# baycom/tfrec

Hardware: AMD Instinct MI355X
Metric: IQ MSamples/s through demod+decode (batched streams) (higher is better)
Workload: dtype int32+f32+f64

## Files before the change

### include/tfrec_amd.h

```cpp
#ifndef TFREC_AMD_H
#define TFREC_AMD_H

#include <stddef.h>
#include <stdint.h>

#ifdef __cplusplus
extern "C" {
#endif

#define TFREC_AMD_BLOCK_BYTES 65536
#define TFREC_AMD_FIFO_DEPTH 4
#define TFREC_AMD_BLOCK_BYTES_10X 655360
#define TFREC_AMD_BLOCK_DEC 8192
#define TFREC_AMD_NSLOTS 5

enum { TFREC_AMD_SLOT_TFA1 = 0, TFREC_AMD_SLOT_TFA2 = 1, TFREC_AMD_SLOT_TFA3 = 2, TFREC_AMD_SLOT_TX22 = 3,
       TFREC_AMD_SLOT_WHB = 4 };

enum {
	TFREC_AMD_OK = 0,
	TFREC_AMD_E_INVAL = -1,
	TFREC_AMD_E_NOMEM = -2,
	TFREC_AMD_E_HIP = -3,
	TFREC_AMD_E_OVERFLOW = -4,
// ... 271 lines not shown
int tfrec_amd_rssi_db(int slot, int64_t rssi_raw);

int tfrec_amd_read_stage0(tfrec_amd_ctx *ctx, int stream, int16_t *out, size_t n_pairs);
int tfrec_amd_read_decimated(tfrec_amd_ctx *ctx, int stream, int16_t *out, size_t n_pairs);
typedef struct {
	uint64_t resolved;
	uint64_t host_verified;
	uint64_t host_mismatch;
	uint64_t undecidable;
	uint64_t reserved[4];
} tfrec_amd_fm_stats;
int tfrec_amd_get_fm_stats(tfrec_amd_ctx *ctx, tfrec_amd_fm_stats *out);
int tfrec_amd_atan_uncertain(tfrec_amd_ctx *ctx, uint64_t *n);
int tfrec_amd_fm_dev_probe(int device, int kind, const void *records, size_t n, int32_t *out, tfrec_amd_fm_stats *stats);
int tfrec_amd_iir_probe(int device, double cutoff, int form, const double *in, size_t n, double *out);
int tfrec_amd_read_biquad_row(tfrec_amd_ctx *ctx, int slot, int stream, int32_t *out, size_t cap_values, uint32_t *n_slots);
int tfrec_amd_get_timings(tfrec_amd_ctx *ctx, tfrec_amd_timings *out);
typedef struct {
	uint64_t biquad_segments;
	uint64_t biquad_unconverged;
	uint64_t biquad_serial;
	uint64_t tfa2_resliced;
	uint64_t tfa1_recomputed;
	uint64_t biquad_repair_slots;
	uint64_t whb_respeculated;
	uint64_t tfa1_scalar_groups;
	uint64_t tfa2_scalar_groups;
	uint64_t tfa1_vector_groups;
	uint64_t tfa2_vector_groups;
} tfrec_amd_stats;
// ... 10 lines not shown
```

### tfrec_amd/api.py

```python
from __future__ import annotations

import ctypes as C
import os
from fractions import Fraction

import numpy as np

from . import _build
from .burst import BURST_DTYPE
from .capture import RUN_DTYPE
from .clock import CLOCK_DTYPE
from .envelope import ENVELOPE_DTYPE
from .levels import LEVEL_DTYPE
from .occupancy import OCC_DTYPE
from .sync import SYNC_DTYPE
from .track import TRACK_DTYPE

BLOCK_BYTES = 65536
BLOCK_DEC = 8192
NSLOTS = 5
FIFO_DEPTH = 4
SLOT_NAMES = ("TFA_1", "TFA_2", "TFA_3", "TX22", "WHB")

F_ALL_FLUSHES = 1
# ... 72 lines not shown
    "tfrec_amd_get_timings", "tfrec_amd_read_thresh", "tfrec_amd_get_stats", "tfrec_amd_get_layout", "tfrec_amd_host_alloc",
    "tfrec_amd_host_free", "tfrec_amd_read_stage0", "tfrec_amd_get_fm_stats", "tfrec_amd_fm_dev_probe",
    "tfrec_amd_fifo_depth", "tfrec_amd_get_memory", "tfrec_amd_iir_probe", "tfrec_amd_reset_streams",
    "tfrec_amd_configure_streams", "tfrec_amd_get_stream_config", "tfrec_amd_tune_streams", "tfrec_amd_get_stream_tune",
    "tfrec_amd_map_streams", "tfrec_amd_get_stream_input", "tfrec_amd_tune_streams_wide", "tfrec_amd_get_stream_tune_wide",
    "tfrec_amd_create_rate", "tfrec_amd_get_input_rate", "tfrec_amd_input_bytes", "tfrec_amd_resample_taps",
    "tfrec_amd_tune_streams_input", "tfrec_amd_get_stream_tune_input", "tfrec_amd_create_format", "tfrec_amd_get_input_format",
    "tfrec_amd_read_levels", "tfrec_amd_enable_capture", "tfrec_amd_read_captures", "tfrec_amd_enable_spectrum",
    "tfrec_amd_read_spectrum", "tfrec_amd_enable_occupancy", "tfrec_amd_read_occupancy", "tfrec_amd_create_dc", "tfrec_amd_get_dc",
    "tfrec_amd_read_dc", "tfrec_amd_reset_dc_rows", "tfrec_amd_create_iq", "tfrec_amd_get_iq", "tfrec_amd_read_iq", "tfrec_amd_reset_iq_rows", "tfrec_amd_create_decimated", "tfrec_amd_enable_capture_pre",
    "tfrec_amd_read_capture_pre", "tfrec_amd_enable_runs_input", "tfrec_amd_submit_runs", "tfrec_amd_read_biquad_row",
    "tfrec_amd_enable_burst_meter", "tfrec_amd_read_bursts", "tfrec_amd_stream_state_bytes", "tfrec_amd_save_streams",
    "tfrec_amd_load_streams", "tfrec_amd_enable_burst_envelope", "tfrec_amd_read_burst_envelopes",
    "tfrec_amd_enable_burst_clock", "tfrec_amd_read_burst_clocks",
    "tfrec_amd_enable_burst_track", "tfrec_amd_set_burst_track_centre", "tfrec_amd_read_burst_tracks",
    "tfrec_amd_enable_burst_sync", "tfrec_amd_read_burst_syncs",
)

_libs = {}


def library_path(experiments: bool = False, short_segments: bool = False) -> str:
    return _build.VARIANTS[_build.variant_name(experiments, short_segments)][0]


def load_library(build: bool = True, experiments: bool = False, short_segments: bool = False):
    key = _build.variant_name(experiments, short_segments)
    if key in _libs:
        return _libs[key]
    if build:
        try:
# ... 23 lines not shown
    L.tfrec_amd_pending_events.argtypes = [C.c_void_p, C.POINTER(C.c_int)]
    L.tfrec_amd_rssi_db.argtypes = [C.c_int, C.c_int64]
    L.tfrec_amd_rssi_db.restype = C.c_int
    L.tfrec_amd_read_decimated.argtypes = [C.c_void_p, C.c_int, C.c_void_p, C.c_size_t]
    L.tfrec_amd_read_stage0.argtypes = [C.c_void_p, C.c_int, C.c_void_p, C.c_size_t]
    L.tfrec_amd_read_biquad_row.argtypes = [C.c_void_p, C.c_int, C.c_int, C.c_void_p, C.c_size_t, C.POINTER(C.c_uint32)]
    L.tfrec_amd_atan_uncertain.argtypes = [C.c_void_p, C.POINTER(C.c_uint64)]
    L.tfrec_amd_get_timings.argtypes = [C.c_void_p, C.POINTER(Timings)]
    L.tfrec_amd_read_thresh.argtypes = [C.c_void_p, C.c_int, C.POINTER(C.c_int)]
    L.tfrec_amd_get_stats.argtypes = [C.c_void_p, C.POINTER(Stats)]
    L.tfrec_amd_get_layout.argtypes = [C.c_void_p, C.POINTER(C.c_int)]
    L.tfrec_amd_get_memory.argtypes = [C.c_void_p, C.POINTER(C.c_uint64), C.POINTER(C.c_uint64)]
    L.tfrec_amd_get_fm_stats.argtypes = [C.c_void_p, C.POINTER(FmStats)]
    L.tfrec_amd_fm_dev_probe.argtypes = [C.c_int, C.c_int, C.c_void_p, C.c_size_t, C.c_void_p, C.POINTER(FmStats)]
    L.tfrec_amd_iir_probe.argtypes = [C.c_int, C.c_double, C.c_int, C.c_void_p, C.c_size_t, C.c_void_p]
    L.tfrec_amd_reset_streams.argtypes = [C.c_void_p, C.c_void_p, C.c_int]
    L.tfrec_amd_configure_streams.argtypes = [C.c_void_p, C.c_void_p, C.c_void_p, C.c_int]
    L.tfrec_amd_get_stream_config.argtypes = [C.c_void_p, C.c_int, C.POINTER(StreamConfig)]
    L.tfrec_amd_tune_streams.argtypes = [C.c_void_p, C.c_void_p, C.c_void_p, C.c_int]
    L.tfrec_amd_get_stream_tune.argtypes = [C.c_void_p, C.c_int, C.POINTER(C.c_int32)]
    L.tfrec_amd_map_streams.argtypes = [C.c_void_p, C.c_void_p, C.c_void_p, C.c_int]
    L.tfrec_amd_get_stream_input.argtypes = [C.c_void_p, C.c_int, C.POINTER(C.c_int32)]
    L.tfrec_amd_tune_streams_wide.argtypes = [C.c_void_p, C.c_void_p, C.c_void_p, C.c_int]
    L.tfrec_amd_get_stream_tune_wide.argtypes = [C.c_void_p, C.c_int, C.POINTER(C.c_int32)]
    L.tfrec_amd_tune_streams_input.argtypes = [C.c_void_p, C.c_void_p, C.c_void_p, C.c_int]
    L.tfrec_amd_get_stream_tune_input.argtypes = [C.c_void_p, C.c_int, C.POINTER(C.c_int32)]
    L.tfrec_amd_create_rate.argtypes = [C.POINTER(Config), C.c_int32, C.c_int32, C.POINTER(C.c_void_p)]
    L.tfrec_amd_get_input_rate.argtypes = [C.c_void_p, C.POINTER(C.c_int32), C.POINTER(C.c_int32)]
    L.tfrec_amd_input_bytes.argtypes = [C.c_void_p, C.c_int, C.POINTER(C.c_size_t)]
    L.tfrec_amd_resample_taps.argtypes = [C.c_int32, C.c_int32, C.c_void_p, C.c_int, C.POINTER(C.c_int)]
# ... 591 lines not shown
    L = load_library()
    q = np.ascontiguousarray(records, dtype=np.int32).reshape(-1, 4)
    out = np.empty(len(q), dtype=np.int32)
    _check(L, L.tfrec_amd_fm_dev_probe(device, 2, q.ctypes.data, len(q), out.ctypes.data, None))
    return out


def iir_probe(cutoff: float, x: np.ndarray, form: int = 1, device: int = 0) -> np.ndarray:
    L = load_library()
    xin = np.ascontiguousarray(x, dtype=np.float64)
    out = np.empty(len(xin), dtype=np.float64)
    _check(L, L.tfrec_amd_iir_probe(device, float(cutoff), int(form), xin.ctypes.data, len(xin), out.ctypes.data))
    return out


def fm_dev_probe(records: np.ndarray, device: int = 0, cross: bool = False):
    L = load_library()
    q = (np.ascontiguousarray(records, dtype=np.int64).reshape(-1, 2) if cross
         else np.ascontiguousarray(records, dtype=np.int32).reshape(-1, 4))
    out = np.empty(len(q), dtype=np.int32)
    st = FmStats()
    _check(L, L.tfrec_amd_fm_dev_probe(device, 1 if cross else 0, q.ctypes.data, len(q), out.ctypes.data, C.byref(st)))
    return out, {n: int(getattr(st, n)) for n, _ in FmStats._fields_[:4]}


def events_canon(events: np.ndarray):
    L = load_library()
    events = events[events["status"] != STATUS_BITS]
    m = np.empty((len(events), 71), dtype=np.int64)
    m[:, 0] = events["slot"]
# ... 47 lines not shown
```

### tfrec_amd/csrc/capi_create.h

```cpp
#pragma once

static BiquadCoef biquad_coef(double cutoff)
{
	static const struct {
		double cutoff, b0, a1, a2;
	} known[] = {
		{ 0.5 / (384000.0 / 17240), 0x1.27f98b1037a14p-8, 0x1.cd1527f4a26e2p+0, -0x1.a36a1c41c6995p-1 },
		{ 0.5 / (384000.0 / 9600), 0x1.7ed02b18a270dp-10, 0x1.e397ac010fc89p+0, -0x1.ca2cf85850d62p-1 },
		{ 0.5 / (384000.0 / 8842), 0x1.461fa1a309718p-10, 0x1.e5d4f47377e30p+0, -0x1.ce36282a35d90p-1 },
		{ 2.0 / 64.0, 0x1.14a67102a1ffdp-7, 0x1.b949652fa3970p+0, -0x1.83dd316f714e0p-1 },
		{ 0.0025 / 64.0, 0x1.02ae4cfc8910ap-26, 0x1.ffe9409fe171bp+0, -0x1.ffd283451f7d3p-1 },
	};
	BiquadCoef c;
	for (const auto &k : known)
		if (k.cutoff == cutoff) {
			c.b0 = k.b0;
			c.b1 = k.b0 + k.b0;
			c.b2 = k.b0;
			c.a1 = k.a1;
			c.a2 = k.a2;
			return c;
		}
	const double i = 1.0 / tan(cutoff * M_PI);
	const double s = sqrt(2.0);
// ... 519 lines not shown
	hipStream_t cp = nullptr;
	TRY(own_stream(c, S.fs, prio_hi));
	TRY(own_stream(c, cp, 0));
	TRY(own_stream(c, S.cs, prio_hi));
	S.ws = S.fs;
	c->cpy = cp;
	if (c->cfg.flags & TFREC_AMD_F_SERIAL_CHAINS)
		return TFREC_AMD_OK;
	TRY(own_stream(c, S.t1, prio_hi));
	TRY(own_stream(c, S.aux, prio_hi));
	const char *dp = TFREC_KNOB_STR("DEEP");
	c->deep = dp ? atoi(dp) != 0 : true;
	c->fmdev_k2 = has_kind(c->launch, 1) && has_kind(c->launch, 2);
	S.k2 = S.cs;
	S.kw = S.aux;
	S.vx = S.aux;
	if (!c->deep)
		return TFREC_AMD_OK;
	TRY(own_stream(c, S.k2, 0));
	TRY(own_stream(c, S.kw, 0));
	S.ws = S.kw;
	if (c->fmdev_k2) {
		TRY(own_stream(c, S.fq, prio_lo));
		TRY(own_stream(c, S.ks, prio_lo));
	}
	TRY(own_stream(c, c->cpy, prio_lo));
	S.vx = cp;
	return TFREC_AMD_OK;
}

static int make_pipes(tfrec_amd_ctx *c, const PipeCtl &S)
{
	const bool serial = (c->cfg.flags & TFREC_AMD_F_SERIAL_CHAINS) != 0;
	const bool timing = (c->cfg.flags & TFREC_AMD_F_TIMING) != 0;
	for (int k = 0; k < kSets; k++) {
		PipeCtl &P = c->pipe[k];
		P = S;
		for (hipEvent_t *e : { &P.done[0], &P.done[1], &P.done[2], &P.ev_win, &P.ev_fork, &P.ev_k2, &P.ev_kw, &P.ev_fm,
				       &P.ev_spec, &c->ev_in[k], &P.ev_front, &c->copied[k] })
			TRY(own_event(c, *e, hipEventDisableTiming));
		if (!serial)
			TRY(own_event(c, P.ev_aux, hipEventDisableTiming));
		if (timing) {
			for (hipEvent_t &e : c->ev[k])
				TRY(own_event(c, e, hipEventDefault));
			if (!serial) {
				for (hipEvent_t &e : c->tev[k])
					TRY(own_event(c, e, hipEventDefault));
				P.tev = c->tev[k];
			}
		}
		P.whb_carry = c->d_whbcarry;
		P.fmdev_wmax = c->fmdev_k2 ? c->wmax : 0;
		P.fm_flag_eps = c->fm_flag_eps;
	}
	return TFREC_AMD_OK;
}
// ... 165 lines not shown
```

### tfrec_amd/csrc/capi_probe.h

```cpp
#pragma once

static void account_fm_log(FmTotals *t, const EventBuf &eb)
{
	t->resolved += eb.uncertain;
	t->undecidable += eb.fm_undecidable;
	const uint32_t n = std::min<uint32_t>(eb.fm_logged, (uint32_t)kFmLogCap);
	const double scale = 16384.0 * (1.0 / M_PI);
	for (uint32_t k = 0; k < n; k++) {
		const int want = d2i_host(atan2(eb.fm_log[k].cj, eb.fm_log[k].cr) * scale);
		t->verified++;
		if (want != eb.fm_log[k].result)
			t->mismatch++;
	}
}

static void report_debug_stats(tfrec_amd_ctx *c, int set, int n_blocks)
{
#ifdef TFREC_AMD_VECSTAT
	if (c->submit_seq == 3) {
		(void)hipDeviceSynchronize();
		unsigned long long st[16] = { 0 };
		(void)hipMemcpy(st, c->win[set].stats, sizeof(st), hipMemcpyDeviceToHost);
		fprintf(stderr, "VECSTAT (one submit) TFA_1: groups %llu, stale piece %llu, entered-with-none hazard %llu, > 64 bits in a lane %llu, lanes with 32 ones or more %llu; TFA_2 family: groups %llu, entered with relative 0 %llu, > 16 rounds %llu, > 64 bits in a lane %llu, walks of the groups that converged %llu\n", st[8], st[9], st[10], st[11], st[5], st[12], st[13], st[14], st[15], st[6]);
	}
// ... 207 lines not shown
		return TFREC_AMD_E_INVAL;
	HIPCHK(hipSetDevice(device));
	double *d_in = nullptr, *d_out = nullptr;
	int rc = TFREC_AMD_OK;
	if (hipMalloc((void **)&d_in, n * 8) != hipSuccess || hipMalloc((void **)&d_out, n * 8) != hipSuccess)
		rc = TFREC_AMD_E_NOMEM;
	if (rc == TFREC_AMD_OK && (hipMemcpy(d_in, in, n * 8, hipMemcpyHostToDevice) != hipSuccess ||
				   launch_iir_probe(nullptr, d_in, n, biquad_coef(cutoff), d_out, form) != hipSuccess ||
				   hipMemcpy(out, d_out, n * 8, hipMemcpyDeviceToHost) != hipSuccess))
		rc = hip_fail(hipGetLastError(), "iir_probe");
	(void)hipFree(d_in);
	(void)hipFree(d_out);
	return rc;
}

int tfrec_amd_read_thresh(tfrec_amd_ctx *c, int stream, int *thresh)
{
	if (!c || !thresh || stream < 0 || stream >= c->cfg.n_streams)
		return TFREC_AMD_E_INVAL;
	if (!c->settings.per_stream && c->cfg.thresh) {
		*thresh = c->cfg.thresh;
		return TFREC_AMD_OK;
	}
	TRY(tfrec_amd_sync(c));
	FskState f;
	HIPCHK(hipMemcpy(&f, c->d_fsk + stream, sizeof(f), hipMemcpyDeviceToHost));
	*thresh = f.thresh;
	return TFREC_AMD_OK;
}

// ... 117 lines not shown
```

### tfrec_amd/csrc/chains2.hip

```cpp
#include <stdlib.h>

#include <algorithm>

#include "decoder_dev.h"
#include "launch.h"
#include <type_traits>
#include "whb_chain_asm.h"

namespace tfrec {

constexpr int kSpecLbi = -(1 << 30);

__device__ __forceinline__ int whb_hook_perturb(const WinTables &T)
{
#ifdef TFREC_AMD_EXPERIMENTS
	return T.whb_test_perturb;
#else
	return 0;
#endif
}
__device__ __forceinline__ int whb_hook_force_fail(const WinTables &T)
{
#ifdef TFREC_AMD_EXPERIMENTS
	return T.whb_force_fail;
// ... 166 lines not shown
					whb_spec = a;
				}
				mark(kMarkWhbDemodEnd, P.aux);
				mark(kMarkWhbDecodeEnd, P.aux);
				mark(kMarkWhbCommitEnd, P.aux);
			}
	}
	if (whb_spec >= 0) {
		if (P.vx != P.aux) {
			TRY(hipEventRecord(P.ev_aux, P.aux));
			TRY(hipStreamWaitEvent(P.vx, P.ev_aux, 0));
		}
		mark(kMarkWhbCheck, P.vx);
		hipLaunchKernelGGL(whb_chain_kernel, dim3((n_streams + kChkStreams - 1) / kChkStreams), dim3(64 * (1 + kChkProducers)), kChkLdsBytes,
				   P.vx, n_streams, L, whb_spec, T);
		hipLaunchKernelGGL(whb_check_kernel, dim3(n_streams), block, 0, P.vx, n_streams, L, whb_spec, T, P.whb_carry);
		ChainLaunch Lr = L;
		WinTables Tr = T;
		Tr.whbpub = L.states[whb_spec];
		Lr.states[whb_spec] = T.whbscr;
		hipLaunchKernelGGL((whb_demod_kernel<true, true>), dim3((n_streams + 63) / 64), block, 64 * 64, P.vx, dec, dec_stride, dev32, n_streams,
				   n_blocks, sample_base, Lr, whb_spec, Tr, events, eb, flags);
		mark(kMarkWhbCheckEnd, P.vx);
		TRY(hipEventRecord(P.done[1], P.vx));
	} else {
		TRY(hipEventRecord(P.done[1], P.aux));
	}
	static_assert(kMarkTfa2End == kMarkTfa2Coop + 3 && kMarkTfa1End == kMarkTfa1Coop + 3, "a slicer chain's marks are consecutive");
	auto slicer_chain = [&](int kind, hipStream_t s_, int m0) {
		if (kind == 0)
			hipLaunchKernelGGL(mark_kernel, dim3(std::max(1, win_blocks / 16)), dim3(256), 0, s_, dec, dec_stride, n_streams,
					   n_blocks, L, T);
		const size_t slds = (kind == 0 ? 8 : 4) * 64 * sizeof(uint4);
		hipLaunchKernelGGL(slicer_kernel, dim3(std::max(64, win_blocks)), block, slds, s_, dec, dec_stride, ld16, n_streams, n_blocks, L, T,
				   lanes, head_chunks, kind, 0);
		mark(m0, s_);
		hipLaunchKernelGGL(coop_slicer_kernel, dim3(coop_blocks), block, 0, s_, dec, dec_stride, ld16, n_streams, n_blocks, L,
				   T, kind);
		mark(m0 + 1, s_);
// ... 56 lines not shown
			TRY(hipStreamWaitEvent(P.t1, P.ev_win, 0));
		mark(kMarkTfa1Slicer, P.t1);
		slicer_chain(0, P.t1, kMarkTfa1Coop);
	}
	TRY(hipEventRecord(P.done[2], P.t1));
#undef TRY
	return hipGetLastError();
}

hipError_t whb_chain_lds_optin()
{
	return hipFuncSetAttribute(reinterpret_cast<const void *>(&whb_chain_kernel), hipFuncAttributeMaxDynamicSharedMemorySize,
				   (int)kChkLdsBytes);
}

}
```

### tfrec_amd/csrc/launch.h

```cpp
#pragma once

namespace tfrec {

struct FrontOut {
	uint32_t *dec;             size_t dec_stride;
	unsigned long long *mask;  size_t mask_stride;
	uint32_t *prevdec;
	int16_t *fmdev;            size_t fmdev_stride;
	int n_streams, n_blocks;
};
struct History {
	const uint8_t *in;
	uint8_t *out;
};
struct RateTable {
	int p, q, t;
	const float *taps;
};
struct CaptureBufs {
	CaptureState *state;
	CaptureStage *stage;
	int stage_cap;
	uint2 *cnt;
	uint4 *base;
// ... 53 lines not shown
hipError_t launch_burst_meter(hipStream_t st, const FrontOut &o, const CaptureBufs &b, tfrec_amd_burst *out);
hipError_t launch_burst_envelope(hipStream_t st, const FrontOut &o, const CaptureBufs &b, tfrec_amd_envelope *out);
hipError_t launch_burst_clock(hipStream_t st, const FrontOut &o, const CaptureBufs &b, tfrec_amd_clock *out);
hipError_t launch_burst_track(hipStream_t st, const FrontOut &o, const CaptureBufs &b, const TrackBufs &k);
hipError_t launch_burst_sync(hipStream_t st, const FrontOut &o, const CaptureBufs &b, const SyncBufs &k);
hipError_t launch_spectrum(hipStream_t st, int fmt, const uint8_t *iq, size_t stride, const SpectrumBufs &b);
hipError_t launch_occupancy(hipStream_t st, const SpectrumBufs &b, uint32_t ratio, uint32_t rel, tfrec_amd_occupancy *recs, uint32_t *bits);
hipError_t launch_fm_probe(hipStream_t st, const int32_t *quads, size_t n, int32_t *out, EventBuf *eb, int kind);
hipError_t launch_iir_probe(hipStream_t st, const double *in, size_t n, const BiquadCoef &c, double *out, int form);
hipError_t launch_chains(hipStream_t st, const FrontOut &o, long long sample_base, const ChainLaunch &L, tfrec_amd_event *events,
			 EventBuf *eb, uint32_t flags);
hipError_t launch_threshold(hipStream_t st, const FrontOut &o, FskState *fsk, int wmax, const StreamCfg *scfg);
hipError_t launch_pipeline(const PipeCtl &P, const FrontOut &o, long long sample_base, const ChainLaunch &L, const WinTables &T, int16_t *ld16,
			   int32_t *dev32, tfrec_amd_event *events, EventBuf *eb, uint32_t flags);
hipError_t whb_chain_lds_optin();
struct StateTable;
hipError_t launch_stream_state(hipStream_t st, bool load, const StateTable &T, const int32_t *list, int n_list, uint8_t *stage);

}
```

### tfrec_amd/csrc/tfrec_dev.h

```cpp
#pragma once

#include <hip/hip_runtime.h>
#include <stddef.h>
#include <stdint.h>

#include "../../include/tfrec_amd.h"

#if defined(__HIP_DEVICE_COMPILE__)
#if !defined(__gfx950__)
#error "tfrec_amd: the device code targets gfx950 (MI355X) only"
#endif
#if defined(__AMDGCN_WAVEFRONT_SIZE) && __AMDGCN_WAVEFRONT_SIZE != 64
#error "tfrec_amd: the device code assumes 64-lane wavefronts"
#endif
#endif

namespace tfrec {

constexpr int kBlockDec = TFREC_AMD_BLOCK_DEC;
constexpr int kIndexSpan = 2 * kBlockDec;
constexpr int kTailBytes = 112;
constexpr int kNSlots = TFREC_AMD_NSLOTS;
constexpr int kFmtU8 = TFREC_AMD_FMT_U8, kFmtS8 = TFREC_AMD_FMT_S8, kFmtS16 = TFREC_AMD_FMT_S16, kFmtF32 = TFREC_AMD_FMT_F32;
constexpr int kFmtDec16 = TFREC_AMD_FMT_DEC16;
// ... 299 lines not shown
	ChainState *whbscr;
	ChainState *whbpub;
	int32_t whb_test_perturb;
	int32_t tfa2_vec;
	int32_t tfa1_vec;
};
constexpr int kStatusDead = 0xff;

struct PipeCtl {
	hipStream_t fs;
	hipStream_t ws;
	hipEvent_t ev_front;
	hipStream_t k2, kw;
	hipStream_t cs, aux, t1;
	hipStream_t vx;
	hipEvent_t ev_aux;
	int *whb_carry;
	hipEvent_t ev_win;
	hipEvent_t ev_fork;
	hipEvent_t ev_k2, ev_kw;
	hipEvent_t ev_fm;
	hipStream_t fq;
	hipStream_t ks;
	hipEvent_t ev_spec;
	hipEvent_t done[3];
	hipEvent_t *tev;
	int fmdev_wmax;
	double fm_flag_eps;
};
enum TimingMark : int {
	kMarkWindows = 0,
// ... 35 lines not shown
```

### tfrec_amd/csrc/whb_check.h

```cpp
#pragma once

#ifndef TFREC_AMD_CHK_STREAMS
#define TFREC_AMD_CHK_STREAMS 32
#endif
constexpr int kChkStreams = TFREC_AMD_CHK_STREAMS;
constexpr int kChkProducers = 2;
constexpr int kChkPerProducer = kChkStreams / kChkProducers;
static_assert(kChkStreams <= 64 && kChkStreams % kChkProducers == 0, "a lane per stream, the streams split evenly");
constexpr int kChkPairRow = 64 * 4 + 4;
constexpr int kChkDevRow = 64 + 4;
struct ChkBuf {
	uint32_t pair[kChkStreams * kChkPairRow];
	uint32_t dev[kChkStreams * kChkDevRow];
};
constexpr size_t kChkLdsBytes = 2 * sizeof(ChkBuf);

__global__ __launch_bounds__(64 * (1 + kChkProducers)) void whb_chain_kernel(int n_streams, ChainLaunch L, int a, WinTables T)
{
	extern __shared__ __attribute__((aligned(16))) uint8_t chk_lds[];
	ChkBuf *const buf = reinterpret_cast<ChkBuf *>(chk_lds);
	const int wave = (int)threadIdx.x >> 6, ln = (int)threadIdx.x & 63;
	const int s0 = (int)blockIdx.x * kChkStreams;
	const ChainParams &p = L.params[a];
	const double a1 = p.iir_avg.a1, a2 = p.iir_avg.a2, bh = 0.5 * p.iir_avg.b0;
	const int my_s = s0 + ln;
	const bool my_on = ln < kChkStreams && my_s < n_streams;
	const int my_rounds = my_on ? T.whbdense_n[my_s] >> 6 : 0;
	int rmax = my_rounds;
#pragma unroll
	for (int o = 32; o >= 1; o >>= 1) {
		const int other = __shfl_xor(rmax, o, 64);
		rmax = other > rmax ? other : rmax;
	}
	rmax = __builtin_amdgcn_readfirstlane(rmax);
	if (rmax == 0)
		return;
	if (wave == 0) {
		double y1 = 0.0, y2 = 0.0;
		if (my_on) {
			const WhbExact st = T.whbx[my_s];
			y1 = st.y1;
			y2 = st.y2;
		}
		unsigned long long *const xbits = T.whbxbits + (size_t)(my_on ? my_s : 0) * T.whbx_stride;
		double2 *const xsnap = T.whbxsnap + (size_t)(my_on ? my_s : 0) * T.whbx_stride;
		__syncthreads();
		for (int r = 0; r < rmax; r++) {
			if (r < my_rounds) {
				const ChkBuf &b = buf[r & 1];
				const double2 *prow = reinterpret_cast<const double2 *>(b.pair + ln * kChkPairRow);
				const uint4 *drow = reinterpret_cast<const uint4 *>(b.dev + ln * kChkDevRow);
				uint32_t acc[2] = { 0u, 0u };
				double2 pq[2][8];
				uint4 dq[2][2];
				auto fetch = [&](int h, int g8) {
#pragma unroll
					for (int j = 0; j < 8; j++)
						pq[h][j] = prow[8 * g8 + j];
					dq[h][0] = drow[2 * g8];
					dq[h][1] = drow[2 * g8 + 1];
// ... 8 lines not shown
							    (int)dq[h][1].x, (int)dq[h][1].y, (int)dq[h][1].z, (int)dq[h][1].w };
#pragma unroll
					for (int j = 0; j < 8; j++) {
						const double P = pq[h][j].x, B2 = pq[h][j].y;
						const double y = ((B2 + a1 * y1) + P) + a2 * y2;
						y2 = y1;
						y1 = y;
						const int yi = (int)y;
						asm("v_cmp_lt_i32 vcc, %1, %2\n\tv_addc_co_u32 %0, vcc, %0, %0, vcc" : "+v"(acc[g8 >> 2]) : "v"(dv[j]), "v"(yi) : "vcc");
					}
				}
				xbits[r] = (unsigned long long)__brev(acc[0]) | ((unsigned long long)__brev(acc[1]) << 32);
				xsnap[r] = make_double2(y1, y2);
			}
			__syncthreads();
		}
	} else {
		const int q0 = (wave - 1) * kChkPerProducer;
		int rounds[kChkPerProducer], h1[kChkPerProducer], h2[kChkPerProducer];
		const int32_t *row[kChkPerProducer];
#pragma unroll
		for (int q = 0; q < kChkPerProducer; q++) {
			const int s = s0 + q0 + q;
			const bool on = s < n_streams;
			rounds[q] = __builtin_amdgcn_readlane(my_rounds, (q0 + q) & 63);
			row[q] = T.whbdense + (size_t)(on ? s : 0) * T.whbdense_stride;
			const WhbExact st = T.whbx[on ? s : 0];
			h1[q] = __builtin_amdgcn_readfirstlane(st.fd1);
			h2[q] = __builtin_amdgcn_readfirstlane(st.fd2);
		}
// ... 9 lines not shown
				if (r < rounds[q]) {
					const int d0 = cur[q];
					const int s1 = __builtin_amdgcn_update_dpp(0, d0, 0x138, 0xf, 0xf, false);
					const int d1 = ln == 0 ? h1[q] : s1;
					const int s2 = __builtin_amdgcn_update_dpp(0, d1, 0x138, 0xf, 0xf, false);
					const int d2 = ln == 0 ? h2[q] : s2;
					const double t0 = bh * (double)d0, t1 = bh * (double)d1, t2 = bh * (double)d2;
					const double P = __builtin_fma(2.0, t1, t0);
					*reinterpret_cast<double2 *>(b.pair + (q0 + q) * kChkPairRow + 4 * ln) = make_double2(P, t2);
					b.dev[(q0 + q) * kChkDevRow + ln] = (uint32_t)d0;
					h1[q] = __builtin_amdgcn_readlane(d0, 63);
					h2[q] = __builtin_amdgcn_readlane(d0, 62);
				}
			}
		};
		lay_out(buf[0], 0);
		__syncthreads();
		for (int r = 0; r < rmax; r++) {
			int far[kChkPerProducer];
#pragma unroll
			for (int q = 0; q < kChkPerProducer; q++)
				far[q] = r + 2 < rounds[q] ? row[q][64 * (r + 2) + ln] : 0;
#pragma unroll
			for (int q = 0; q < kChkPerProducer; q++)
				cur[q] = nxt[q];
			if (r + 1 < rmax)
				lay_out(buf[(r + 1) & 1], r + 1);
#pragma unroll
			for (int q = 0; q < kChkPerProducer; q++)
				nxt[q] = far[q];
			__syncthreads();
		}
	}
}

constexpr int kChkLockCap = 256;
__global__ __launch_bounds__(64) void whb_check_kernel(int n_streams, ChainLaunch L, int a, WinTables T, int *__restrict__ carry_io)
{
	__shared__ int lk_pos[kChkLockCap], lk_avgf[kChkLockCap];
	__shared__ uint32_t lk_meta[kChkLockCap];
	const int s = (int)blockIdx.x, ln = (int)threadIdx.x;
	if (s >= n_streams)
		return;
	const ChainParams &p = L.params[a];
	const double a1 = p.iir_avg.a1, a2 = p.iir_avg.a2, bh = 0.5 * p.iir_avg.b0;
	const int N = T.whbdense_n[s], R = N >> 6;
	const int32_t *dense = T.whbdense + (size_t)s * T.whbdense_stride;
	const unsigned long long *xbits = T.whbxbits + (size_t)s * T.whbx_stride;
	const double2 *xsnap = T.whbxsnap + (size_t)s * T.whbx_stride;
	const WhbExact st0 = T.whbx[s];
	const int tp_ = whb_hook_perturb(T);
	const int tol = tp_ > 1 ? tp_ : (tp_ < -1 ? -tp_ : 1);
	auto input = [&](int pos) -> int { return pos >= 0 ? dense[pos] : (pos == -1 ? st0.fd1 : st0.fd2); };
	auto run = [&](int rr, int cnt, double &y1, double &y2, unsigned long long &bits) {
		const int p0 = 64 * rr;
		if (rr == 0) {
			y1 = st0.y1;
			y2 = st0.y2;
		} else {
			const double2 sn = xsnap[rr - 1];
			y1 = sn.x;
			y2 = sn.y;
		}
		double t1 = bh * (double)input(p0 - 1), t2 = bh * (double)input(p0 - 2);
		bits = 0ull;
		for (int k = 0; k < cnt; k++) {
			const int d = dense[p0 + k];
			const double t0 = bh * (double)d;
			const double P = __builtin_fma(2.0, t1, t0);
			const double y = ((t2 + a1 * y1) + P) + a2 * y2;
			bits |= (unsigned long long)(d < (int)y ? 1u : 0u) << k;
			y2 = y1;
			y1 = y;
			t2 = t1;
			t1 = t0;
		}
	};
	double yf1 = 0.0, yf2 = 0.0;
	unsigned long long tailbits = 0ull;
	if (ln == 0)
		run(R, N & 63, yf1, yf2, tailbits);
	tailbits = __shfl(tailbits, 0, 64);
	auto word = [&](int i) -> unsigned long long { return i < R ? xbits[i] : (i == R ? tailbits : 0ull); };
	const uint4 *recrow = reinterpret_cast<const uint4 *>(T.whbrec + (size_t)s * T.whbrec_stride);
	int carry = carry_io[s];
	const int carry_in = carry;
	bool bad = false;
	int cbase = 0, nlocks = 0;
	bool ended = false;
	int last_delta = 0;
	bool have_last = false, last_closed = false;
	auto do_locks = [&]() {
		for (int b0 = 0; b0 < nlocks; b0 += 64) {
			const int i = b0 + ln;
			const bool on = i < nlocks;
			double y1 = 0.0, y2 = 0.0;
			unsigned long long bits;
			const int pos = on ? lk_pos[i] : 0;
			run(pos >> 6, on ? (pos & 63) + 1 : 0, y1, y2, bits);
			const uint32_t meta = on ? lk_meta[i] : 0u;
			const int delta = (int)y1 - (on ? lk_avgf[i] : 0);
			const bool b = on && (delta > tol || delta < -tol || (delta != 0 && (meta & kWhbRecAmb)));
			bad = bad || __ballot(b) != 0ull;
			const int nb = nlocks - b0 < 64 ? nlocks - b0 : 64;
			last_delta = __shfl(delta, nb - 1, 64);
			last_closed = (__shfl((int)meta, nb - 1, 64) & (int)kWhbRecClosed) != 0;
			have_last = true;
		}
		nlocks = 0;
	};
	for (int v0 = 0; !ended; v0 += 64) {
		const int vi = v0 + ln < T.whbrec_stride - 1 ? v0 + ln : T.whbrec_stride - 1;
		const uint4 rec = recrow[vi];
		const uint32_t meta = rec.z;
		const unsigned long long endm = __ballot(meta == kWhbRecEnd);
		const int nrec = endm ? __builtin_ctzll(endm) : 64;
		ended = endm != 0ull || v0 + 64 + 64 > T.whbrec_stride;
		const bool on = ln < nrec;
		const bool pseudo = on && (meta & kWhbRecPseudo) != 0u;
		const bool normal = on && !pseudo;
		const int nv = normal ? (int)((meta >> kWhbRecNvShift) & 63u) + 1 : 0;
		int inc = nv;
#pragma unroll
		for (int o = 1; o < 64; o <<= 1) {
			const int up = __shfl_up(inc, o, 64);
			inc += ln >= o ? up : 0;
		}
		const int pos0 = cbase + inc - nv;
		cbase += __shfl(inc, 63, 64);
		if (pseudo) {
			if (v0 + ln == 0) {
				bad = bad || (carry != 0 && (meta & kWhbRecAmb));
// ... 20 lines not shown
				const int i = nlocks + __builtin_popcountll(lm & ((1ull << ln) - 1ull));
				lk_pos[i] = pos0 + nv - 1;
				lk_avgf[i] = (int)rec.w;
				lk_meta[i] = meta;
			}
			nlocks += __builtin_popcountll(lm);
			__syncthreads();
		}
	}
	if (nlocks)
		do_locks();
	bad = __ballot(bad) != 0ull || cbase != N;
	if (have_last)
		carry = last_closed ? 0 : last_delta;
	if (ln == 0) {
		WhbExact st = st0;
		st.carry = carry_in;
		st.pad_ = 0;
		T.whbx0[s] = st;
		bad = bad || T.whbseen[s] != T.whbgen[s];
		if (whb_hook_force_fail(T) > 0 && (s + T.whb_submit_seq) % whb_hook_force_fail(T) == 0)
			bad = true;
		st.y1 = yf1;
		st.y2 = yf2;
		st.fd1 = input(N - 1);
		st.fd2 = input(N - 2);
		st.carry = st.pad_ = 0;
		T.whbx[s] = st;
		carry_io[s] = bad ? 0 : carry;
		T.whbfail[s] = bad ? 1 : 0;
	}
}
```

Measured before the change: 308,000.

## Move WHB tail recursion into chain kernel and allow check on separate stream

The chain kernel now processes the partial final 64-sample group of each WHB stream, writes its tail bits and end state, and saves the start state in whbx0. This removes the serial lane-0 tail loop and state writeback from the check kernel. An optional knob can place the check and demod kernels on a separate or copy stream behind an event, so they may overlap with other work. A probe entry point is added for testing the chain kernel. The default stream placement is unchanged, so only the moved tail computation affects the default path.

```diff
diff --git a/include/tfrec_amd.h b/include/tfrec_amd.h
--- a/include/tfrec_amd.h
+++ b/include/tfrec_amd.h
@@ -309,6 +309,9 @@
 int tfrec_amd_atan_uncertain(tfrec_amd_ctx *ctx, uint64_t *n);
 int tfrec_amd_fm_dev_probe(int device, int kind, const void *records, size_t n, int32_t *out, tfrec_amd_fm_stats *stats);
 int tfrec_amd_iir_probe(int device, double cutoff, int form, const double *in, size_t n, double *out);
+int tfrec_amd_whb_chain_probe(int device, int n_streams, int stride, double a1, double a2, double b0, const int32_t *seq,
+			      const int32_t *n, const double *y_start, const int32_t *fd_start, uint64_t *bits, double *snap,
+			      double *y_end, int32_t *fd_end, double *y_seen, int32_t *fd_seen);
 int tfrec_amd_read_biquad_row(tfrec_amd_ctx *ctx, int slot, int stream, int32_t *out, size_t cap_values, uint32_t *n_slots);
 int tfrec_amd_get_timings(tfrec_amd_ctx *ctx, tfrec_amd_timings *out);
 typedef struct {
diff --git a/tfrec_amd/api.py b/tfrec_amd/api.py
--- a/tfrec_amd/api.py
+++ b/tfrec_amd/api.py
@@ -110,7 +110,7 @@
     "tfrec_amd_load_streams", "tfrec_amd_enable_burst_envelope", "tfrec_amd_read_burst_envelopes",
     "tfrec_amd_enable_burst_clock", "tfrec_amd_read_burst_clocks",
     "tfrec_amd_enable_burst_track", "tfrec_amd_set_burst_track_centre", "tfrec_amd_read_burst_tracks",
-    "tfrec_amd_enable_burst_sync", "tfrec_amd_read_burst_syncs",
+    "tfrec_amd_enable_burst_sync", "tfrec_amd_read_burst_syncs", "tfrec_amd_whb_chain_probe",
 )
 
 _libs = {}
@@ -164,6 +164,8 @@
     L.tfrec_amd_get_fm_stats.argtypes = [C.c_void_p, C.POINTER(FmStats)]
     L.tfrec_amd_fm_dev_probe.argtypes = [C.c_int, C.c_int, C.c_void_p, C.c_size_t, C.c_void_p, C.POINTER(FmStats)]
     L.tfrec_amd_iir_probe.argtypes = [C.c_int, C.c_double, C.c_int, C.c_void_p, C.c_size_t, C.c_void_p]
+    if hasattr(L, "tfrec_amd_whb_chain_probe"):
+        L.tfrec_amd_whb_chain_probe.argtypes = [C.c_int, C.c_int, C.c_int, C.c_double, C.c_double, C.c_double] + [C.c_void_p] * 10
     L.tfrec_amd_reset_streams.argtypes = [C.c_void_p, C.c_void_p, C.c_int]
     L.tfrec_amd_configure_streams.argtypes = [C.c_void_p, C.c_void_p, C.c_void_p, C.c_int]
     L.tfrec_amd_get_stream_config.argtypes = [C.c_void_p, C.c_int, C.POINTER(StreamConfig)]
@@ -785,6 +787,23 @@
     return out
 
 
+def whb_chain_probe(seq: np.ndarray, n: np.ndarray, y_start: np.ndarray, fd_start: np.ndarray, a1: float, a2: float, b0: float,
+                    device: int = 0) -> dict:
+    L = load_library()
+    q = np.ascontiguousarray(seq, dtype=np.int32)
+    ns, stride = q.shape
+    nn = np.ascontiguousarray(n, dtype=np.int32).reshape(ns)
+    y0 = np.ascontiguousarray(y_start, dtype=np.float64).reshape(ns, 2)
+    f0 = np.ascontiguousarray(fd_start, dtype=np.int32).reshape(ns, 2)
+    out = {"bits": np.zeros((ns, stride // 64), np.uint64), "snap": np.zeros((ns, stride // 64, 2), np.float64),
+           "y_end": np.zeros((ns, 2), np.float64), "fd_end": np.zeros((ns, 2), np.int32),
+           "y_seen": np.zeros((ns, 2), np.float64), "fd_seen": np.zeros((ns, 2), np.int32)}
+    _check(L, L.tfrec_amd_whb_chain_probe(device, ns, stride, float(a1), float(a2), float(b0), q.ctypes.data, nn.ctypes.data,
+                                          y0.ctypes.data, f0.ctypes.data, *(out[k].ctypes.data for k in
+                                                                           ("bits", "snap", "y_end", "fd_end", "y_seen", "fd_seen"))))
+    return out
+
+
 def fm_dev_probe(records: np.ndarray, device: int = 0, cross: bool = False):
     L = load_library()
     q = (np.ascontiguousarray(records, dtype=np.int64).reshape(-1, 2) if cross
diff --git a/tfrec_amd/csrc/capi_create.h b/tfrec_amd/csrc/capi_create.h
--- a/tfrec_amd/csrc/capi_create.h
+++ b/tfrec_amd/csrc/capi_create.h
@@ -557,7 +557,7 @@
 	c->fmdev_k2 = has_kind(c->launch, 1) && has_kind(c->launch, 2);
 	S.k2 = S.cs;
 	S.kw = S.aux;
-	S.vx = S.aux;
+	S.vx = S.vr = S.aux;
 	if (!c->deep)
 		return TFREC_AMD_OK;
 	TRY(own_stream(c, S.k2, 0));
@@ -568,7 +568,12 @@
 		TRY(own_stream(c, S.ks, prio_lo));
 	}
 	TRY(own_stream(c, c->cpy, prio_lo));
-	S.vx = cp;
+	S.vx = S.vr = cp;
+	const int vr_where = has_kind(c->launch, 2) ? TFREC_KNOB_INT("WHB_CHECK_STREAM", 0, 0, 2) : 0;
+	if (vr_where == 2)
+		TRY(own_stream(c, S.vr, prio_lo));
+	else if (vr_where == 1)
+		S.vr = c->cpy;
 	return TFREC_AMD_OK;
 }
 
@@ -582,8 +587,10 @@
 		for (hipEvent_t *e : { &P.done[0], &P.done[1], &P.done[2], &P.ev_win, &P.ev_fork, &P.ev_k2, &P.ev_kw, &P.ev_fm,
 				       &P.ev_spec, &c->ev_in[k], &P.ev_front, &c->copied[k] })
 			TRY(own_event(c, *e, hipEventDisableTiming));
-		if (!serial)
+		if (!serial) {
 			TRY(own_event(c, P.ev_aux, hipEventDisableTiming));
+			TRY(own_event(c, P.ev_chain, hipEventDisableTiming));
+		}
 		if (timing) {
 			for (hipEvent_t &e : c->ev[k])
 				TRY(own_event(c, e, hipEventDefault));
diff --git a/tfrec_amd/csrc/capi_probe.h b/tfrec_amd/csrc/capi_probe.h
--- a/tfrec_amd/csrc/capi_probe.h
+++ b/tfrec_amd/csrc/capi_probe.h
@@ -245,6 +245,57 @@
 	return rc;
 }
 
+int tfrec_amd_whb_chain_probe(int device, int n_streams, int stride, double a1, double a2, double b0, const int32_t *seq,
+			      const int32_t *n, const double *y_start, const int32_t *fd_start, uint64_t *bits, double *snap,
+			      double *y_end, int32_t *fd_end, double *y_seen, int32_t *fd_seen)
+{
+	if (!seq || !n || !y_start || !fd_start || !bits || !snap || !y_end || !fd_end || !y_seen || !fd_seen || n_streams < 1 ||
+	    n_streams > (1 << 16) || stride < 64 || stride > (1 << 20) || stride % 64)
+		return TFREC_AMD_E_INVAL;
+	const size_t ns = (size_t)n_streams, words = (size_t)stride / 64;
+	for (size_t s = 0; s < ns; s++)
+		if (n[s] < 0 || n[s] > stride - 64)
+			return TFREC_AMD_E_INVAL;
+	HIPCHK(hipSetDevice(device));
+	std::vector<WhbExact> hx(ns);
+	for (size_t s = 0; s < ns; s++)
+		hx[s] = WhbExact{ y_start[2 * s], y_start[2 * s + 1], fd_start[2 * s], fd_start[2 * s + 1], 0, 0 };
+	WinTables T = {};
+	T.whbdense_stride = stride;
+	T.whbx_stride = (int32_t)words;
+	int rc = TFREC_AMD_OK;
+	if (hipMalloc((void **)&T.whbdense, ns * (size_t)stride * 4) != hipSuccess || hipMalloc((void **)&T.whbdense_n, ns * 4) != hipSuccess ||
+	    hipMalloc((void **)&T.whbx, ns * sizeof(WhbExact)) != hipSuccess || hipMalloc((void **)&T.whbx0, ns * sizeof(WhbExact)) != hipSuccess ||
+	    hipMalloc((void **)&T.whbxbits, ns * words * 8) != hipSuccess || hipMalloc((void **)&T.whbxsnap, ns * words * 16) != hipSuccess)
+		rc = TFREC_AMD_E_NOMEM;
+	std::vector<WhbExact> hx0(ns);
+	if (rc == TFREC_AMD_OK &&
+	    (hipMemcpy(T.whbdense, seq, ns * (size_t)stride * 4, hipMemcpyHostToDevice) != hipSuccess ||
+	     hipMemcpy(T.whbdense_n, n, ns * 4, hipMemcpyHostToDevice) != hipSuccess ||
+	     hipMemcpy(T.whbx, hx.data(), ns * sizeof(WhbExact), hipMemcpyHostToDevice) != hipSuccess ||
+	     hipMemset(T.whbx0, 0xff, ns * sizeof(WhbExact)) != hipSuccess || hipMemset(T.whbxbits, 0, ns * words * 8) != hipSuccess ||
+	     hipMemset(T.whbxsnap, 0, ns * words * 16) != hipSuccess ||
+	     launch_whb_chain_probe(nullptr, n_streams, a1, a2, b0, T) != hipSuccess ||
+	     hipMemcpy(bits, T.whbxbits, ns * words * 8, hipMemcpyDeviceToHost) != hipSuccess ||
+	     hipMemcpy(snap, T.whbxsnap, ns * words * 16, hipMemcpyDeviceToHost) != hipSuccess ||
+	     hipMemcpy(hx.data(), T.whbx, ns * sizeof(WhbExact), hipMemcpyDeviceToHost) != hipSuccess ||
+	     hipMemcpy(hx0.data(), T.whbx0, ns * sizeof(WhbExact), hipMemcpyDeviceToHost) != hipSuccess))
+		rc = hip_fail(hipGetLastError(), "whb_chain_probe");
+	for (size_t s = 0; s < ns && rc == TFREC_AMD_OK; s++) {
+		y_end[2 * s] = hx[s].y1, y_end[2 * s + 1] = hx[s].y2;
+		fd_end[2 * s] = hx[s].fd1, fd_end[2 * s + 1] = hx[s].fd2;
+		y_seen[2 * s] = hx0[s].y1, y_seen[2 * s + 1] = hx0[s].y2;
+		fd_seen[2 * s] = hx0[s].fd1, fd_seen[2 * s + 1] = hx0[s].fd2;
+	}
+	(void)hipFree(T.whbdense);
+	(void)hipFree(T.whbdense_n);
+	(void)hipFree(T.whbx);
+	(void)hipFree(T.whbx0);
+	(void)hipFree(T.whbxbits);
+	(void)hipFree(T.whbxsnap);
+	return rc;
+}
+
 int tfrec_amd_read_thresh(tfrec_amd_ctx *c, int stream, int *thresh)
 {
 	if (!c || !thresh || stream < 0 || stream >= c->cfg.n_streams)
diff --git a/tfrec_amd/csrc/chains2.hip b/tfrec_amd/csrc/chains2.hip
--- a/tfrec_amd/csrc/chains2.hip
+++ b/tfrec_amd/csrc/chains2.hip
@@ -204,15 +204,19 @@
 		mark(kMarkWhbCheck, P.vx);
 		hipLaunchKernelGGL(whb_chain_kernel, dim3((n_streams + kChkStreams - 1) / kChkStreams), dim3(64 * (1 + kChkProducers)), kChkLdsBytes,
 				   P.vx, n_streams, L, whb_spec, T);
-		hipLaunchKernelGGL(whb_check_kernel, dim3(n_streams), block, 0, P.vx, n_streams, L, whb_spec, T, P.whb_carry);
+		if (P.vr != P.vx) {
+			TRY(hipEventRecord(P.ev_chain, P.vx));
+			TRY(hipStreamWaitEvent(P.vr, P.ev_chain, 0));
+		}
+		hipLaunchKernelGGL(whb_check_kernel, dim3(n_streams), block, 0, P.vr, n_streams, L, whb_spec, T, P.whb_carry);
 		ChainLaunch Lr = L;
 		WinTables Tr = T;
 		Tr.whbpub = L.states[whb_spec];
 		Lr.states[whb_spec] = T.whbscr;
-		hipLaunchKernelGGL((whb_demod_kernel<true, true>), dim3((n_streams + 63) / 64), block, 64 * 64, P.vx, dec, dec_stride, dev32, n_streams,
+		hipLaunchKernelGGL((whb_demod_kernel<true, true>), dim3((n_streams + 63) / 64), block, 64 * 64, P.vr, dec, dec_stride, dev32, n_streams,
 				   n_blocks, sample_base, Lr, whb_spec, Tr, events, eb, flags);
-		mark(kMarkWhbCheckEnd, P.vx);
-		TRY(hipEventRecord(P.done[1], P.vx));
+		mark(kMarkWhbCheckEnd, P.vr);
+		TRY(hipEventRecord(P.done[1], P.vr));
 	} else {
 		TRY(hipEventRecord(P.done[1], P.aux));
 	}
@@ -299,4 +303,20 @@
 				   (int)kChkLdsBytes);
 }
 
-}
+hipError_t launch_whb_chain_probe(hipStream_t st, int n_streams, double a1, double a2, double b0, const WinTables &T)
+{
+	ChainLaunch L = {};
+	L.n_active = 1;
+	L.params[0].kind = 2;
+	L.params[0].iir_avg.a1 = a1;
+	L.params[0].iir_avg.a2 = a2;
+	L.params[0].iir_avg.b0 = b0;
+	const hipError_t e = whb_chain_lds_optin();
+	if (e != hipSuccess)
+		return e;
+	hipLaunchKernelGGL(whb_chain_kernel, dim3((n_streams + kChkStreams - 1) / kChkStreams), dim3(64 * (1 + kChkProducers)), kChkLdsBytes, st,
+			   n_streams, L, 0, T);
+	return hipGetLastError();
+}
+
+}
diff --git a/tfrec_amd/csrc/launch.h b/tfrec_amd/csrc/launch.h
--- a/tfrec_amd/csrc/launch.h
+++ b/tfrec_amd/csrc/launch.h
@@ -91,6 +91,7 @@
 hipError_t launch_pipeline(const PipeCtl &P, const FrontOut &o, long long sample_base, const ChainLaunch &L, const WinTables &T, int16_t *ld16,
 			   int32_t *dev32, tfrec_amd_event *events, EventBuf *eb, uint32_t flags);
 hipError_t whb_chain_lds_optin();
+hipError_t launch_whb_chain_probe(hipStream_t st, int n_streams, double a1, double a2, double b0, const WinTables &T);
 struct StateTable;
 hipError_t launch_stream_state(hipStream_t st, bool load, const StateTable &T, const int32_t *list, int n_list, uint8_t *stage);
 
diff --git a/tfrec_amd/csrc/tfrec_dev.h b/tfrec_amd/csrc/tfrec_dev.h
--- a/tfrec_amd/csrc/tfrec_dev.h
+++ b/tfrec_amd/csrc/tfrec_dev.h
@@ -337,7 +337,9 @@
 	hipStream_t k2, kw;
 	hipStream_t cs, aux, t1;
 	hipStream_t vx;
+	hipStream_t vr;
 	hipEvent_t ev_aux;
+	hipEvent_t ev_chain;
 	int *whb_carry;
 	hipEvent_t ev_win;
 	hipEvent_t ev_fork;
diff --git a/tfrec_amd/csrc/whb_check.h b/tfrec_amd/csrc/whb_check.h
--- a/tfrec_amd/csrc/whb_check.h
+++ b/tfrec_amd/csrc/whb_check.h
@@ -25,25 +25,31 @@
 	const double a1 = p.iir_avg.a1, a2 = p.iir_avg.a2, bh = 0.5 * p.iir_avg.b0;
 	const int my_s = s0 + ln;
 	const bool my_on = ln < kChkStreams && my_s < n_streams;
-	const int my_rounds = my_on ? T.whbdense_n[my_s] >> 6 : 0;
-	int rmax = my_rounds;
+	const int my_n = my_on ? T.whbdense_n[my_s] : 0;
+	const int my_rounds = my_n >> 6, my_tail = my_n & 63;
+	int nmax = my_n;
 #pragma unroll
 	for (int o = 32; o >= 1; o >>= 1) {
-		const int other = __shfl_xor(rmax, o, 64);
-		rmax = other > rmax ? other : rmax;
-	}
-	rmax = __builtin_amdgcn_readfirstlane(rmax);
-	if (rmax == 0)
+		const int other = __shfl_xor(nmax, o, 64);
+		nmax = other > nmax ? other : nmax;
+	}
+	nmax = __builtin_amdgcn_readfirstlane(nmax);
+	const int rmax = nmax >> 6;
+	WhbExact st = { 0.0, 0.0, 0, 0, 0, 0 };
+	if (wave == 0 && my_on) {
+		st = T.whbx[my_s];
+		st.carry = st.pad_ = 0;
+		T.whbx0[my_s] = st;
+	}
+	if (nmax == 0)
 		return;
 	if (wave == 0) {
-		double y1 = 0.0, y2 = 0.0;
-		if (my_on) {
-			const WhbExact st = T.whbx[my_s];
-			y1 = st.y1;
-			y2 = st.y2;
-		}
+		double y1 = st.y1, y2 = st.y2;
 		unsigned long long *const xbits = T.whbxbits + (size_t)(my_on ? my_s : 0) * T.whbx_stride;
 		double2 *const xsnap = T.whbxsnap + (size_t)(my_on ? my_s : 0) * T.whbx_stride;
+		const int32_t *const my_row = T.whbdense + (size_t)(my_on ? my_s : 0) * T.whbdense_stride;
+		const int end1 = my_n >= 1 ? my_row[my_n - 1] : st.fd1;
+		const int end2 = my_n >= 2 ? my_row[my_n - 2] : (my_n == 1 ? st.fd1 : st.fd2);
 		__syncthreads();
 		for (int r = 0; r < rmax; r++) {
 			if (r < my_rounds) {
@@ -82,6 +88,27 @@
 				xsnap[r] = make_double2(y1, y2);
 			}
 			__syncthreads();
+		}
+		if (my_tail) {
+			const ChkBuf &b = buf[rmax & 1];
+			const double2 *prow = reinterpret_cast<const double2 *>(b.pair + ln * kChkPairRow);
+			const uint32_t *drow = b.dev + ln * kChkDevRow;
+			unsigned long long bits = 0ull;
+			for (int k = 0; k < my_tail; k++) {
+				const double2 pq = prow[k];
+				const double y = ((pq.y + a1 * y1) + pq.x) + a2 * y2;
+				y2 = y1;
+				y1 = y;
+				bits |= (unsigned long long)((int)drow[k] < (int)y ? 1u : 0u) << k;
+			}
+			xbits[my_rounds] = bits;
+		}
+		if (my_on && my_n > 0) {
+			st.y1 = y1;
+			st.y2 = y2;
+			st.fd1 = end1;
+			st.fd2 = end2;
+			T.whbx[my_s] = st;
 		}
 	} else {
 		const int q0 = (wave - 1) * kChkPerProducer;
@@ -121,7 +148,30 @@
 				}
 			}
 		};
-		lay_out(buf[0], 0);
+		auto lay_rests = [&](ChkBuf &b) {
+#pragma unroll
+			for (int q = 0; q < kChkPerProducer; q++) {
+				const int tail = __builtin_amdgcn_readlane(my_tail, (q0 + q) & 63);
+				if (tail > 0) {
+					const int d0 = ln < tail ? row[q][64 * rounds[q] + ln] : 0;
+					const int s1 = __builtin_amdgcn_update_dpp(0, d0, 0x138, 0xf, 0xf, false);
+					const int d1 = ln == 0 ? h1[q] : s1;
+					const int s2 = __builtin_amdgcn_update_dpp(0, d1, 0x138, 0xf, 0xf, false);
+					const int d2 = ln == 0 ? h2[q] : s2;
+					const double t0 = bh * (double)d0, t1 = bh * (double)d1, t2 = bh * (double)d2;
+					const double P = __builtin_fma(2.0, t1, t0);
+					if (ln < tail) {
+						*reinterpret_cast<double2 *>(b.pair + (q0 + q) * kChkPairRow + 4 * ln) = make_double2(P, t2);
+						b.dev[(q0 + q) * kChkDevRow + ln] = (uint32_t)d0;
+					}
+				}
+				asm volatile("" ::: "memory");
+			}
+		};
+		if (rmax > 0)
+			lay_out(buf[0], 0);
+		else
+			lay_rests(buf[0]);
 		__syncthreads();
 		for (int r = 0; r < rmax; r++) {
 			int far[kChkPerProducer];
@@ -133,6 +183,8 @@
 				cur[q] = nxt[q];
 			if (r + 1 < rmax)
 				lay_out(buf[(r + 1) & 1], r + 1);
+			else
+				lay_rests(buf[(r + 1) & 1]);
 #pragma unroll
 			for (int q = 0; q < kChkPerProducer; q++)
 				nxt[q] = far[q];
@@ -151,11 +203,11 @@
 		return;
 	const ChainParams &p = L.params[a];
 	const double a1 = p.iir_avg.a1, a2 = p.iir_avg.a2, bh = 0.5 * p.iir_avg.b0;
-	const int N = T.whbdense_n[s], R = N >> 6;
+	const int N = T.whbdense_n[s];
 	const int32_t *dense = T.whbdense + (size_t)s * T.whbdense_stride;
 	const unsigned long long *xbits = T.whbxbits + (size_t)s * T.whbx_stride;
 	const double2 *xsnap = T.whbxsnap + (size_t)s * T.whbx_stride;
-	const WhbExact st0 = T.whbx[s];
+	const WhbExact st0 = T.whbx0[s];
 	const int tp_ = whb_hook_perturb(T);
 	const int tol = tp_ > 1 ? tp_ : (tp_ < -1 ? -tp_ : 1);
 	auto input = [&](int pos) -> int { return pos >= 0 ? dense[pos] : (pos == -1 ? st0.fd1 : st0.fd2); };
@@ -183,12 +235,8 @@
 			t1 = t0;
 		}
 	};
-	double yf1 = 0.0, yf2 = 0.0;
-	unsigned long long tailbits = 0ull;
-	if (ln == 0)
-		run(R, N & 63, yf1, yf2, tailbits);
-	tailbits = __shfl(tailbits, 0, 64);
-	auto word = [&](int i) -> unsigned long long { return i < R ? xbits[i] : (i == R ? tailbits : 0ull); };
+	const int W = (N + 63) >> 6;
+	auto word = [&](int i) -> unsigned long long { return i < W ? xbits[i] : 0ull; };
 	const uint4 *recrow = reinterpret_cast<const uint4 *>(T.whbrec + (size_t)s * T.whbrec_stride);
 	int carry = carry_io[s];
 	const int carry_in = carry;
@@ -216,13 +264,13 @@
 		}
 		nlocks = 0;
 	};
-	for (int v0 = 0; !ended; v0 += 64) {
+	for (int v0 = 0; !ended && v0 < T.whbrec_stride; v0 += 64) {
 		const int vi = v0 + ln < T.whbrec_stride - 1 ? v0 + ln : T.whbrec_stride - 1;
 		const uint4 rec = recrow[vi];
 		const uint32_t meta = rec.z;
 		const unsigned long long endm = __ballot(meta == kWhbRecEnd);
 		const int nrec = endm ? __builtin_ctzll(endm) : 64;
-		ended = endm != 0ull || v0 + 64 + 64 > T.whbrec_stride;
+		ended = endm != 0ull;
 		const bool on = ln < nrec;
 		const bool pseudo = on && (meta & kWhbRecPseudo) != 0u;
 		const bool normal = on && !pseudo;
@@ -273,19 +321,10 @@
 	if (have_last)
 		carry = last_closed ? 0 : last_delta;
 	if (ln == 0) {
-		WhbExact st = st0;
-		st.carry = carry_in;
-		st.pad_ = 0;
-		T.whbx0[s] = st;
+		T.whbx0[s].carry = carry_in;
 		bad = bad || T.whbseen[s] != T.whbgen[s];
 		if (whb_hook_force_fail(T) > 0 && (s + T.whb_submit_seq) % whb_hook_force_fail(T) == 0)
 			bad = true;
-		st.y1 = yf1;
-		st.y2 = yf2;
-		st.fd1 = input(N - 1);
-		st.fd2 = input(N - 2);
-		st.carry = st.pad_ = 0;
-		T.whbx[s] = st;
 		carry_io[s] = bad ? 0 : carry;
 		T.whbfail[s] = bad ? 1 : 0;
 	}
```

Result: no change. 308,700, median of 6 (+0.2%).
